# lyndonchan/wsss-analysis

Measured on AMD Instinct MI355X. Metric: images/sec CAM+CRF pseudo-labels, VOC2012 321x321, higher is better.
Workload: dtype f16x3; 1 GPU; resnet50 CAM + dense-CRF (M=21, 10 mean-field iters), 321x321, batch 32 images (=64 samples) per GPU, image-sharded; batch_images=32, num_classes=20, parallelism=image-sharded x1, no collective, steps_per_rank=239

## Files before the change

include/wsscam.h:

```cpp
#ifndef WSSCAM_H
#define WSSCAM_H

#include <stddef.h>
#include <stdint.h>

#ifdef __cplusplus
extern "C" {
#endif

#define WSC_VERSION 100

typedef enum wsc_status {
    WSC_OK = 0,
    WSC_ERR_INVALID = -1,
    WSC_ERR_NO_DEVICE = -2,
    WSC_ERR_HIP = -3,
    WSC_ERR_MISSING_KEY = -4,
    WSC_ERR_SHAPE = -5,
    WSC_ERR_NOMEM = -6,
    WSC_ERR_KEY_RANGE = -7,
    WSC_ERR_CAPACITY = -8,
    WSC_ERR_RANGE = -9
} wsc_status;

// ... 17 lines not shown
} wsc_precision;

typedef struct wsc_ctx wsc_ctx;
typedef struct wsc_net wsc_net;
typedef enum {
    WSC_OPT_CRF_GAUSS_ON_CHIP = 0,
    WSC_OPT_CRF_FUSED_BLUR = 1,
    WSC_OPT_CRF_BLUR_ON_CHIP = 2,
    WSC_OPT_CRF_RANK_BALLOT = 3,
    WSC_OPT_CRF_EMBED_FULL = 4,
    WSC_OPT_RW_TILED = 5,
    WSC_OPT_STEM_POOL_FUSED = 6,
    WSC_OPT_CONV_WINDOW = 7,
    WSC_OPT_CAM_HEAD_STREAM = 8,
    WSC_OPT_CRF_MSG_IN_UPDATE = 9,
    WSC_OPT_COUNT = 10
} wsc_option;

typedef struct wsc_crf wsc_crf;
typedef struct wsc_crf_v wsc_crf_v;

typedef struct wsc_tensor_desc {
    const char *name;
    const float *data;
    int32_t ndim;
    int64_t shape[4];
} wsc_tensor_desc;


int wsc_version(void);
const char *wsc_last_error(void);
// ... 384 lines not shown
```

profiles/conv_layer_table.py:

```python
import re
import sqlite3
import sys


def resnet50_layers(S):
    def o(h, k, s, p):
        return (h + 2 * p - k) // s + 1

    L = []
    h = o(S, 7, 2, 3)
    L.append(("stem 7x7 s2 3->64", h, 3, 64, 7))
    h = o(h, 3, 2, 1)
    inp = 64
    for li, (planes, blocks, stride) in enumerate(((64, 3, 1), (128, 4, 2), (256, 6, 2), (512, 3, 1)), 1):
        for b in range(blocks):
            s = stride if b == 0 else 1
            ho = o(h, 3, s, 1)
            n = "layer%d.%d." % (li, b)
            L.append((n + "conv1 1x1 %d->%d" % (inp, planes), h, inp, planes, 1))
            L.append((n + "conv2 3x3 %d s%d" % (planes, s), ho, planes, planes, 3))
            if b == 0:
                L.append((n + "conv3+proj 1x1 (%d+%d)->%d" % (planes, inp, planes * 4), ho, planes + inp, planes * 4, 1))
            else:
                L.append((n + "conv3 1x1 %d->%d +res" % (planes, planes * 4), ho, planes, planes * 4, 1))
# ... 17 lines not shown
def main(db, N=64, S=321, planes=1):
    c = sqlite3.connect(db)
    tabs = [r[0] for r in c.execute("select name from sqlite_master where type='table'")]
    kd = [t for t in tabs if "kernel_dispatch" in t][0]
    ks = [t for t in tabs if "kernel_symbol" in t][0]
    rows = c.execute("select s.kernel_name, d.start, d.end, d.grid_size_x / d.workgroup_size_x, d.group_segment_size "
                     "from %s d join %s s on d.kernel_id = s.id order by d.start" % (kd, ks)).fetchall()
    start = [i for i, r in enumerate(rows) if "nchw_to_nhwc4" in r[0]][-1]
    convs = [r for r in rows[start:] if "conv_igemm_kernel" in r[0] or "stem_pool_kernel" in r[0] or "cam_head_kernel" in r[0]]
    layers = resnet50_layers(S)
    if "stem_pool_kernel" in convs[0][0]:
        layers[0] = ("stem 7x7 s2 3->64 + maxpool (fused)",) + layers[0][1:]
    print("%-44s %8s %8s %9s %7s %6s" % ("layer", "us", "TFLOP/s", "act TB/s", "blocks", "LDS KB"))
    tot = 0.0
    pos = 0
    for (name, ho, cin, cout, k) in layers:
        M = N * ho * ho
        nd = n_dispatches(M, cin, cout, k, planes=planes)
        rs = convs[pos:pos + nd]
        pos += nd
        us = sum(r[2] - r[1] for r in rs) / 1000.0
        tot += us
        fl = 2.0 * M * cout * k * k * cin
        by = 2.0 * M * cout * (2 if "+res" in name else 1) + 2.0 * N * (ho * (2 if "s2" in name else 1)) ** 2 * cin
        if "fused" in name:
            by = 8.0 * N * S * S + 2.0 * N * ((ho + 1) // 2) ** 2 * cout
        by *= planes
        print("%-44s %8.1f %8.0f %9.2f %7s %6s" % (name, us, fl / us / 1e6, by / us / 1e6, "+".join(str(r[3]) for r in rs),
                                                    "/".join("%.0f" % (r[4] / 1024.0) for r in rs)))
    print("conv kernels total %.1f us" % tot)


if __name__ == "__main__":
    main(sys.argv[1], *(int(v) for v in sys.argv[2:]))
```

wsss-analysis_amd/csrc/common.h:

```cpp
#pragma once
#include <hip/hip_runtime.h>
#include <assert.h>
#include <stdint.h>
#include <map>
#include <string>
#include <unordered_map>
#include <vector>

#include "../../include/wsscam.h"

typedef uint16_t bf16_t;

typedef __bf16 bf16x8_t __attribute__((ext_vector_type(8)));
typedef _Float16 f16x8_t __attribute__((ext_vector_type(8)));
typedef float f32x16_t __attribute__((ext_vector_type(16)));
typedef float f32x4_t __attribute__((ext_vector_type(4)));

__host__ __device__ inline bf16_t f32_to_bf16(float f) {
    union { float f; uint32_t u; } v;
    v.f = f;
    uint32_t u = v.u;
    if ((u & 0x7fffffffu) > 0x7f800000u) return (bf16_t)((u >> 16) | 0x40);
    u += 0x7fffu + ((u >> 16) & 1u);
    return (bf16_t)(u >> 16);
// ... 106 lines not shown
    hipStream_t stream = nullptr;
    bool own_stream = false;
    int num_cus = 0;
    std::string arch;
    void *ws = nullptr;
    size_t ws_bytes = 0;
    static constexpr int PIN_SLOTS = 8;
    struct PinSlot {
        void *p = nullptr;
        size_t bytes = 0;
        hipEvent_t ev = nullptr;
        bool busy = false;
    };
    PinSlot pin_ring[PIN_SLOTS];
    int pin_next = 0;
    int opt[WSC_OPT_COUNT] = {1, 1, 1, 0, 0, -1, 1, 1, 1, 1};
    void *zero_page = nullptr;
    unsigned *range_host = nullptr, *range_dev = nullptr;
    hipEvent_t ev0 = nullptr, ev1 = nullptr;
    hipEvent_t join_ev = nullptr;
    hipEvent_t marks[8] = {};
    bool mark_set[8] = {};
    hipStream_t aux_stream = nullptr;
    hipEvent_t fork_ev = nullptr, aux_done_ev = nullptr;
    bool profiling = false;
    std::vector<WscProfRecord> prof;
    std::vector<hipEvent_t> prof_pool;
    std::multimap<size_t, void *> free_blocks;
    std::unordered_map<void *, size_t> live_blocks;
    WscGaussCache *gauss_cache = nullptr;
    int scratch_fill = -1;
// ... 182 lines not shown
    const float *s1, *b1;
    const float *s2, *b2;
    Act res;
    Act y;
    float *y_f32;
    int N, H, W, Cin, Ho, Wo, Cout, CoutPad;
    int kh, kw, stride, pad;
    int dil = 1;
    int relu;
    ConvForm form;
    wsc_precision prec;
    int generic;
    int ldy;
    Act x2;
    int H2, W2, C2, stride2;
    bool operands_match() const {
        for (const Act *a : {&x, &res, &y, &x2})
            if (*a && a->prec != prec) return false;
        return true;
    }
};
int conv_igemm_launch(wsc_ctx *ctx, const ConvLaunch &p);
int conv_f32_launch(wsc_ctx *ctx, const ConvLaunch &p);
int launch_cam_head(wsc_ctx *ctx, Act x, int M, int K, const bf16_t *w, int Kw, int CoutPad, const float *s1, const float *b1,
                    int C, int relu, float *y);

inline int wsc_grid_for(long long total, int block = 256, int cap = 256 * 16) {
    long long g = (total + block - 1) / block;
    if (g > cap) g = cap;
    if (g < 1) g = 1;
    return (int)g;
}
inline unsigned *layer_door(wsc_ctx *ctx, wsc_precision prec) { return conv_fmt(prec) == 1 ? ctx->range_dev : nullptr; }
int launch_nchw_to_nhwc4(wsc_ctx *ctx, const float *x, int N, int H, int W, Act y, unsigned *range);
void stem_pool_input_dims(int H, int W, int *Hp, int *Wp);
int launch_stem_pool(wsc_ctx *ctx, Act x, int N, int H, int W, const bf16_t *w, int Kw, const float *s1, const float *b1, int relu,
                     Act y);
// ... 141 lines not shown
```

wsss-analysis_amd/csrc/conv_igemm.hip:

```cpp
#include "common.h"

#include <type_traits>

namespace {

constexpr int BK = 64;

struct ConvKArgs {
    const bf16_t *x, *x_lo, *w;
    const float *s1, *b1, *s2, *b2;
    const bf16_t *res, *res_lo;
    bf16_t *y, *y_lo;
    float *y_f32;
    int H, W, Cin, Ho, Wo, Cout;
    int ldy;
    int kh, kw, stride, pad, relu;
    int M, HoWo;
    int m_base, m_end;
    unsigned div_howo_mul, div_howo_s1, div_howo_s2, div_wo_mul, div_wo_s1, div_wo_s2;
    int cchunks;
    int dil;
    int ksteps_base;
    int nk;
    int Kw;
    int Kbase;
    int ntiles_n, nblocks;
    const bf16_t *zero;
    int spare1;
    long long lo_delta;
    const bf16_t *x2;
    long long lo_delta2;
    int cc2, H2, W2, C2, stride2;
    int ldx;
    int win_npix;
    int spare2, spare3;
    unsigned *range;
};

__device__ __forceinline__ int lds_off(int row, int slot) {
    return row * 128 + ((slot ^ ((row >> 1) & 7)) << 4);
}

__device__ __forceinline__ void decode_row(const ConvKArgs &p, int m, int &n, int &ho, int &wo) {
    const unsigned t1 = __umulhi(p.div_howo_mul, (unsigned)m);
    n = (int)((t1 + (((unsigned)m - t1) >> p.div_howo_s1)) >> p.div_howo_s2);
    const int rem = m - n * p.HoWo;
    const unsigned t2 = __umulhi(p.div_wo_mul, (unsigned)rem);
    ho = (int)((t2 + (((unsigned)rem - t2) >> p.div_wo_s1)) >> p.div_wo_s2);
    wo = rem - ho * p.Wo;
}

template <int BM, int BN, int MODE, int SPLIT, int ET, int STAGES, int FAST = 0, int WPT = 0>
__global__ __launch_bounds__(BM * 2, (STAGES == 1 && FAST != 0) ? 4 : 2) void conv_igemm_kernel(ConvKArgs p) {
    constexpr bool GLDS = MODE == 0;
    constexpr int WMT = BM == 256 ? 128 : 64;
    constexpr bool FEPI = (FAST & 1) != 0, PW = (FAST & 2) != 0;
    constexpr bool WIN = WPT > 0;
    static_assert(!WIN || (SPLIT == 2 && BM == 128 && STAGES == 2 && FAST == 1), "LDS window: single-staged split, 128-row tile");
    static_assert(FAST == 0 || (SPLIT != 1 && ET == 1 && (MODE == 0 || FAST == 1)),
                  "FAST paths: f16, one plane or the single-staged split; the pointwise prologue belongs to the LDS-DMA layers");
    static_assert(SPLIT != 2 || (MODE == 0 && STAGES == 2), "single-staged split: LDS-DMA layers, two LDS buffers");
    static_assert(STAGES == 2 || SPLIT == 0, "one LDS buffer serves a one-K-step layer, which a layer of three K segments never is");
    constexpr int CK = SPLIT == 2 ? 32 : 64;
    constexpr int NT = BM * 2;
    constexpr int NW = BM / 32;
    constexpr int WR = BM / WMT;
    constexpr int WC = NW / WR;
    constexpr int WN = BN / WC;
// ... 516 lines not shown
        }
    } else {
        load_tile(0);
        store_lds(0);
        __syncthreads();
        for (int kt = 0; kt < nk; ++kt) {
            const int cur = kt & 1;
            const bool more = kt + 1 < nk;
            if (more) load_tile(kt + 1);
            compute(cur);
            if (more) store_lds(cur ^ 1);
            __syncthreads();
        }
    }

    constexpr int TPR = BN / 8;
    constexpr int RPP = NT / TPR;
    constexpr int NPASS = BM / RPP;
    const int c8 = t % TPR;
    const int r0 = t / TPR;
    const int c = n0 + c8 * 8;
    const bool cok = c < p.Cout;
    const bool full = c + 8 <= p.Cout;
    const bool has_res = p.res != nullptr && full;
    constexpr bool PRE_ALL = WMT == 64 && !(STAGES == 1 && FEPI);
    constexpr int NHALF_R = STAGES == 1 ? BM / 64 : (WMT == 128 ? BM / 128 : 1);
    constexpr int NRES = PRE_ALL ? NPASS : NPASS / NHALF_R;
    uint4 rres[NRES], rres_lo[NRES];
    auto fetch_res = [&](int first_pass) {
#pragma unroll
// ... 190 lines not shown
                    if (SPLIT) *reinterpret_cast<uint4 *>(p.y_lo + oy) = make_uint4(lw[0], lw[1], lw[2], lw[3]);
                }
            }
        }
    }
    if (ET && (ovf & 0x80008000u)) *p.range = (unsigned)p.Cout;
}

typedef void (*ConvKernel)(ConvKArgs);
struct ConvVariant {
    ConvKernel kernel;
    int bm, bn;
    int lds;
    int cls;
};
template <int BM, int BN, int MODE, int SPLIT, int ET, int STAGES, int FAST = 0, int WPT = 0>
ConvVariant variant() {
    constexpr int A_BYTES = BM * BK * 2, B_BYTES = BN * BK * 2;
    constexpr int PIPE = WPT > 0 ? WPT * 4096 + STAGES * B_BYTES : STAGES * (A_BYTES + B_BYTES);
    constexpr int EPI = (STAGES == 1 ? 64 : (BM == 256 ? 128 : BM)) * (BN + 4) * 4;
    constexpr int LDS = PIPE > EPI ? PIPE : EPI;
    static_assert(LDS <= 160 * 1024, "LDS budget of a CU");
    return {conv_igemm_kernel<BM, BN, MODE, SPLIT, ET, STAGES, FAST, WPT>, BM, BN, LDS,
            MODE != 0 ? WSC_K_CONV_SMALLCIN : (BM == 256 ? WSC_K_CONV256 : (BN == 128 ? WSC_K_CONV128 : WSC_K_CONV64))};
}
template <int BM, int BN, int MODE, int ET, int FAST = 0>
ConvVariant one_plane(bool one_kstep) {
    if constexpr (BM == 128)
        if (one_kstep) return variant<BM, BN, MODE, 0, ET, 1, FAST>();
    return variant<BM, BN, MODE, 0, ET, 2, FAST>();
}
template <int BM, int BN>
ConvVariant select_variant(ConvForm form, wsc_precision prec, int fast, bool one_kstep, int wpt) {
    if constexpr (BM == 128) {
        auto small = [&](auto mode) {
            constexpr int MODE = decltype(mode)::value;
            switch (prec) {
            case WSC_PREC_BF16: return one_plane<128, BN, MODE, 0>(one_kstep);
            case WSC_PREC_BF16X3: return variant<128, BN, MODE, 1, 0, 2>();
            case WSC_PREC_F16: return fast ? one_plane<128, BN, MODE, 1, 1>(one_kstep) : one_plane<128, BN, MODE, 1>(one_kstep);
            default: return variant<128, BN, MODE, 1, 1, 2>();
            }
        };
        if (form == CONV_FORM_SMALL2) return small(std::integral_constant<int, 1>{});
        if (form == CONV_FORM_SMALL4) return small(std::integral_constant<int, 2>{});
        if (wpt == 8) return variant<128, BN, 0, 2, 1, 2, 1, 8>();
        if (wpt == 10) return variant<128, BN, 0, 2, 1, 2, 1, 10>();
    }
    ConvVariant v;
    switch (prec) {
    case WSC_PREC_BF16: v = one_plane<BM, BN, 0, 0>(one_kstep); break;
    case WSC_PREC_BF16X3: v = variant<BM, BN, 0, 1, 0, 2>(); break;
    case WSC_PREC_F16:
        v = fast == 3 ? one_plane<BM, BN, 0, 1, 3>(one_kstep) : (fast ? one_plane<BM, BN, 0, 1, 1>(one_kstep) : one_plane<BM, BN, 0, 1>(one_kstep));
        break;
    default:
        v = fast == 3 ? variant<BM, BN, 0, 2, 1, 2, 3>() : (fast ? variant<BM, BN, 0, 2, 1, 2, 1>() : variant<BM, BN, 0, 2, 1, 2>());
        break;
    }
    if (form == CONV_FORM_STEM_ROWS) v.cls = WSC_K_CONV_SMALLCIN;
    return v;
}
ConvVariant conv_variant(int bm, int bn, ConvForm form, wsc_precision prec, int fast, bool one_kstep, int wpt = 0) {
    if (bm == 256) return select_variant<256, 256>(form, prec, fast, one_kstep, wpt);
    return bn == 128 ? select_variant<128, 128>(form, prec, fast, one_kstep, wpt) : select_variant<128, 64>(form, prec, fast, one_kstep, wpt);
}

}

int conv_igemm_launch(wsc_ctx *ctx, const ConvLaunch &p) {
    if (p.prec == WSC_PREC_F32) return conv_f32_launch(ctx, p);
    WSC_CHECK(p.operands_match(), WSC_ERR_INVALID, "conv: an operand is not of the layer's precision %d", (int)p.prec);
    const int split = conv_split(p.prec), fmt = conv_fmt(p.prec);
    const bool dma = conv_form_dma(p.form);
    if (p.form == CONV_FORM_STEM_ROWS)
        WSC_CHECK(split == 2 && p.Cin == 4 && p.pad == 0 && p.kw <= 7 && (p.stride & 1) == 0, WSC_ERR_INVALID,
                  "conv: the padded-stem form needs split 2, a 4-channel padded input, kw <= 7 and an even stride");
    else if (p.form == CONV_FORM_GENERIC) WSC_CHECK(p.Cin % 64 == 0, WSC_ERR_INVALID, "conv: Cin=%d not a multiple of 64", p.Cin);
    else WSC_CHECK(p.Cin == 4, WSC_ERR_INVALID, "conv: small-Cin mode needs a 4-channel activation");
    const ConvKLayout k = conv_k_layout(p.kh, p.kw, p.Cin, p.form, p.prec);
    const bool single_staged = k.interleaved;
    ConvKArgs a = {};
// ... 6 lines not shown
    a.win_npix = 0;
    a.ldx = p.Cin; a.x2 = nullptr; a.lo_delta2 = 0; a.cc2 = 0; a.H2 = a.W2 = a.C2 = 0; a.stride2 = 1;
    a.kh = p.kh; a.kw = k.kw_steps; a.stride = p.stride; a.pad = p.pad; a.relu = p.relu;
    a.M = p.N * p.Ho * p.Wo;
    a.HoWo = p.Ho * p.Wo;
    conv_fastdiv((unsigned)(a.HoWo > 0 ? a.HoWo : 1), &a.div_howo_mul, &a.div_howo_s1, &a.div_howo_s2);
    conv_fastdiv((unsigned)(p.Wo > 0 ? p.Wo : 1), &a.div_wo_mul, &a.div_wo_s1, &a.div_wo_s2);
    WSC_CHECK(p.dil >= 1, WSC_ERR_INVALID, "conv: dilation %d", p.dil);
    const int dil = (p.kh == 1 && p.kw == 1) ? 1 : p.dil;
    WSC_CHECK(dil == 1 || (p.form == CONV_FORM_GENERIC && !p.x2), WSC_ERR_INVALID,
              "conv: dilation %d needs a generic layer (Cin %% 64 == 0) with one input", dil);
    a.dil = dil;
    a.cchunks = k.cchunks; a.ksteps_base = k.ksteps_base;
    a.Kbase = k.Kbase; a.Kw = k.Kw; a.nk = k.nk;
    a.lo_delta = single_staged ? (long long)(a.x_lo - a.x) : 0;
    if (p.x2) {
        const int K1 = p.Cin - p.C2;
        WSC_CHECK(split != 1 && dma && p.kh == 1 && p.kw == 1 && p.stride == 1 && p.pad == 0 && K1 > 0 &&
                  K1 % 64 == 0 && p.C2 % 64 == 0 && p.stride2 >= 1 && (p.Ho - 1) * p.stride2 < p.H2 && (p.Wo - 1) * p.stride2 < p.W2 &&
                  (!single_staged || p.x2.h16_lo() != nullptr),
                  WSC_ERR_INVALID, "conv: a second input needs a 1x1 / stride 1 layer, channel counts in multiples of 64 and no bf16x3");
        a.x2 = p.x2.h16();
        a.lo_delta2 = single_staged ? (long long)(p.x2.h16_lo() - a.x2) : 0;
        a.cc2 = K1 / k.ck;
        a.H2 = p.H2; a.W2 = p.W2; a.C2 = p.C2; a.stride2 = p.stride2;
        a.ldx = K1;
    }
    WSC_CHECK(p.CoutPad % 64 == 0, WSC_ERR_INVALID, "conv: CoutPad=%d not a multiple of 64", p.CoutPad);
    const int BN = conv_tile_bn(p.CoutPad);
    a.zero = (const bf16_t *)ctx->zero_page;
    a.range = ctx->range_dev;
    int fast = 0;
    if (!p.generic && dil == 1 && fmt && (split == 0 || single_staged) && p.y && p.y_f32 == nullptr &&
        p.Cout == p.CoutPad && (long long)a.M * a.ldy < (1ll << 31)) {
        fast = 1;
        if (dma && p.kh == 1 && p.kw == 1 && p.pad == 0 && p.stride == 1) fast = 3;
    }
    if (a.M == 0) return WSC_OK;
    auto launch = [&](const ConvVariant &v, int m_base, int m_end) -> int {
        ConvKArgs b = a;
        b.m_base = m_base;
        b.m_end = m_end;
        b.ntiles_n = p.CoutPad / v.bn;
        b.nblocks = ((m_end - m_base + v.bm - 1) / v.bm) * b.ntiles_n;
        WSC_TRY(wsc_set_max_dynamic_lds(ctx, reinterpret_cast<const void *>(v.kernel), v.lds));
        const double flops = 2.0 * (m_end - m_base) * a.Cout * (p.form == CONV_FORM_GENERIC ? (double)p.kh * p.kw * p.Cin : (double)p.kh * p.kw * 3);
        WscKernelTimer timer(ctx, v.cls, flops);
        hipLaunchKernelGGL(v.kernel, dim3(b.nblocks), dim3(v.bm * 2), v.lds, ctx->stream, b);
        WSC_HIP(hipGetLastError());
        return WSC_OK;
    };
    const bool one_kstep = a.nk == 1;
    const long long blocks_sq = ((a.M + 255) / 256) * (long long)(p.CoutPad / 256);
    bool square = dma && p.CoutPad % 256 == 0 && a.nk >= 4 && blocks_sq >= 192;
    if (split == 2 && !fast) square = false;
    if (split == 2 && a.nk < 16) square = false;
    if (square) {
        const ConvVariant sq = conv_variant(256, 256, p.form, p.prec, fast, one_kstep);
        const long long rounds = blocks_sq / ctx->num_cus, rem = blocks_sq - rounds * ctx->num_cus;
        if (rounds >= 1 && rem > 0 && rem * 2 <= ctx->num_cus && ctx->num_cus > 0) {
            const int big_rows = (int)((rounds * ctx->num_cus) / (p.CoutPad / 256));
            WSC_TRY(launch(sq, 0, big_rows * 256));
            return launch(conv_variant(128, BN, p.form, p.prec, fast, one_kstep), big_rows * 256, a.M);
        }
        return launch(sq, 0, a.M);
    }
    int wpt = 0;
    if (single_staged && fast == 1 && dil == 1 && p.kh == 3 && p.kw == 3 && p.stride == 1 && p.pad == 1 && !p.x2 &&
        p.Ho == p.H && p.Wo == p.W && ctx->opt[WSC_OPT_CONV_WINDOW] != 0) {
        const long long need = 127 + 2ll * p.W + 3 + 1;
        const long long npix = (long long)p.N * p.H * p.W;
        if (need <= 320 && npix < (1ll << 30) && a.lo_delta >= 0 && npix * p.Cin + a.lo_delta < (1ll << 33) && (a.lo_delta & 7) == 0) {
            a.win_npix = (int)npix;
            wpt = need <= 256 ? 8 : 10;
        }
    }
    return launch(conv_variant(128, BN, p.form, p.prec, fast, one_kstep, wpt), 0, a.M);
}
```

wsss-analysis_amd/csrc/net.hip:

```cpp
#include "common.h"

#include <algorithm>
#include <cmath>
#include <cstring>
#include <unordered_map>

namespace {

struct HostTensor {
    const float *data;
    int ndim;
    int64_t shape[4];
    int64_t numel() const {
        int64_t n = 1;
        for (int i = 0; i < ndim; ++i) n *= shape[i];
        return n;
    }
};
typedef std::unordered_map<std::string, HostTensor> Dict;

struct ConvW {
    void *w = nullptr;
    float *s1 = nullptr, *b1 = nullptr, *s2 = nullptr, *b2 = nullptr;
    int Cin = 0, Cout = 0, CoutPad = 0, kh = 1, kw = 1, stride = 1, pad = 0, relu = 0;
// ... 723 lines not shown
}

bool stem_pool_fused(const wsc_ctx *ctx, const wsc_net *net) {
    if (net->ops.empty() || net->ops[0].type != OP_CONV || net->ops[0].in >= 0 || net->convs[net->ops[0].conv].form != CONV_FORM_STEM_ROWS)
        return false;
    const ConvW &c0 = net->convs[net->ops[0].conv];
    bool tapped = false;
    for (int tp : net->taps) tapped = tapped || tp == 0;
    return ctx->opt[WSC_OPT_STEM_POOL_FUSED] && net->ops.size() > 1 && net->ops[1].type == OP_POOL &&
           net->ops[1].in == net->ops[0].out && net->ops[1].rule == POOL_TORCH && !net->ops[1].avg && net->ops[1].pk == 3 &&
           net->ops[1].ps == 2 && net->ops[1].pp == 1 &&
           c0.kh == 7 && c0.kw == 7 && c0.stride == 2 && c0.pad == 3 && c0.Cout == 64 && c0.s2 == nullptr &&
           net->ops[0].res < 0 && conv_fmt(net->prec) == 1 && !tapped;
}

struct TraceSink {
    const long long *off;
    float *out;
};

int run_backbone(wsc_ctx *ctx, const wsc_net *net, const float *x_dev, int N, int S, size_t extra_bytes, Act *feat, int *hf, int *wf,
                 void **extra, std::vector<Act> *taps = nullptr, int SW = 0, bool nhwc_in = false, Act *spare = nullptr,
                 const TraceSink *trace = nullptr, Act *xin_out = nullptr) {
    if (SW <= 0) SW = S;
    Plan pl;
    WSC_TRY(plan_dims(net, N, S, SW, &pl));
    int in_h = S, in_w = SW, in_pad = 0;
    bool fused_stem = false;
    if (!net->ops.empty() && net->ops[0].type == OP_CONV && net->ops[0].in < 0 && net->convs[net->ops[0].conv].form == CONV_FORM_STEM_ROWS) {
        const ConvW &c0 = net->convs[net->ops[0].conv];
// ... 9 lines not shown
    void *ws;
    WSC_TRY(wsc_ctx_workspace(ctx, act_bytes(in_elems, net->prec) + 4 * act_bytes(pl.max_act, net->prec) + align_up(extra_bytes, 256), &ws));
    char *p = (char *)ws;
    const Act xin = act_carve(p, in_elems, net->prec);
    Act buf[4];
    for (Act &b : buf) b = act_carve(p, pl.max_act, net->prec);
    if (taps)
        for (int op : net->taps) taps->push_back(act_carve(p, pl.out_elems(N, op), net->prec));
    *extra = (void *)p;

    if (nhwc_in) {
        WSC_CHECK(in_pad == 0, WSC_ERR_INVALID, "internal: an NHWC input has no padded-stem form");
        WSC_TRY(launch_nhwc3_to_nhwc4(ctx, x_dev, N, S, SW, xin));
    } else if (in_pad > 0) WSC_TRY(launch_nchw_to_nhwc4_pad(ctx, x_dev, N, S, SW, in_h, in_w, in_pad, xin, ctx->range_dev));
    else WSC_TRY(launch_nchw_to_nhwc4(ctx, x_dev, N, S, SW, xin, ctx->range_dev));
    for (size_t i = 0; i < net->ops.size(); ++i) {
        const Op &op = net->ops[i];
        const OpDims &d = pl.ops[i];
        const Act src = op.in < 0 ? xin : buf[op.in];
        if (fused_stem && i == 0) continue;
        if (fused_stem && i == 1) {
            const ConvW &c0 = net->convs[net->ops[0].conv];
            WSC_TRY(launch_stem_pool(ctx, xin, N, S, SW, (const bf16_t *)c0.w, conv_k_layout(c0.kh, c0.kw, c0.Cin, c0.form, net->prec).Kw, c0.s1,
                                     c0.b1, c0.relu, buf[op.out]));
        } else if (op.type == OP_CONV) {
            const ConvW &c = net->convs[op.conv];
            ConvLaunch L = conv_launch(c, net->prec);
            L.x = src;
            if (op.res >= 0) L.res = buf[op.res];
            L.y = buf[op.out].at(op.coff);
            L.ldy = op.pitch;
            if (op.in2 >= 0) {
                L.x2 = buf[op.in2];
                L.H2 = d.H2; L.W2 = d.W2; L.C2 = d.C2; L.stride2 = op.ps;
            }
            L.N = N; L.H = d.H; L.W = d.W; L.Ho = d.Ho; L.Wo = d.Wo;
            if (c.form == CONV_FORM_STEM_ROWS && op.in < 0) on_padded_input(L, in_h, in_w);
            WSC_TRY(conv_igemm_launch(ctx, L));
        } else if (op.type == OP_GATHER) {
            WSC_TRY(launch_gather_strided(ctx, src, N, d.H, d.W, d.C, op.ps, d.Ho, d.Wo, buf[op.out].at(op.coff), op.pitch));
        } else {
            PoolGeom g;
            WSC_CHECK(pool_geom(op.rule, op.pk, op.ps, op.pp, op.avg, d.H, d.W, &g), WSC_ERR_INVALID, "internal: a pool plan_dims let through");
            WSC_TRY(launch_pool(ctx, src, N, d.H, d.W, d.C, g, buf[op.out]));
        }
        if (trace && trace->off[i] >= 0) WSC_TRY(launch_act_to_f32(ctx, buf[op.out], pl.out_elems(N, (int)i), trace->out + trace->off[i]));
        if (taps)
            for (size_t k = 0; k < net->taps.size(); ++k)
                if (net->taps[k] == (int)i) {
                    const size_t nb = pl.out_elems(N, (int)i) * conv_elem_bytes(net->prec);
                    WSC_HIP(hipMemcpyAsync((*taps)[k].hi, buf[op.out].hi, nb, hipMemcpyDeviceToDevice, ctx->stream));
                    if (buf[op.out].lo) WSC_HIP(hipMemcpyAsync((*taps)[k].lo, buf[op.out].lo, nb, hipMemcpyDeviceToDevice, ctx->stream));
                }
    }
    *feat = buf[net->final_buf];
    if (xin_out) *xin_out = xin;
    if (spare) *spare = buf[net->final_buf == 3 ? 2 : 3];
    *hf = pl.hf;
    *wf = pl.wf;
    return WSC_OK;
}

int run_classifier(wsc_ctx *ctx, const wsc_net *net, Act feat, Act spare, int N, int count, int sample_stride, int hf, int wf,
                   float *score_dev) {
    int hw = hf * wf;
    if (net->cls_max && net->cls_pool_set) {
        const PoolSpec &ps = net->cls_pool;
        PoolGeom g;
// ... 176 lines not shown
        const OpDims &d = pl->ops[i];
        wsc_trace_op t = {};
        set_label(t, op.label);
        t.in = producer(op.in);
        t.in2 = t.res = WSC_TRACE_NONE;
        t.Ho = d.Ho; t.Wo = d.Wo; t.pitch = d.Co; t.coff = op.coff; t.C = d.Co;
        if (op.type == OP_CONV) {
            const ConvW &c = net->convs[op.conv];
            t.kind = WSC_TRACE_CONV;
            t.C = c.Cout;
            if (op.in2 >= 0) t.in2 = producer(op.in2);
            if (op.res >= 0) t.res = producer(op.res);
            t.kh = c.kh; t.kw = c.kw; t.stride = c.stride; t.pad = c.pad; t.dil = c.dil; t.relu = c.relu;
            t.affine2 = c.s2 != nullptr;
            t.stride2 = op.in2 >= 0 ? op.ps : 0;
            t.fused_next = fused && i == 0;
        } else if (op.type == OP_GATHER) {
            t.kind = WSC_TRACE_GATHER;
            t.C = d.C;
            t.stride = op.ps;
        } else {
            t.kind = WSC_TRACE_POOL;
            t.pool_rule = (int)op.rule; t.pool_k = op.pk; t.pool_stride = op.ps; t.pool_pad = op.pp; t.pool_avg = op.avg;
        }
        writer[op.out] = (int)i;
        out->push_back(t);
    }
    if (net->head.w != nullptr) {
        wsc_trace_op t = {};
        set_label(t, "head");
        t.kind = WSC_TRACE_HEAD;
// ... 1210 lines not shown
```

wsss-analysis_amd/wsscam/_lib.py:

```python
import ctypes
import os
import re
import threading

import numpy as np

_HERE = os.path.dirname(os.path.abspath(__file__))
LIB_PATH = os.path.join(_HERE, "libwsscam.so")
HEADER_PATH = os.path.normpath(os.path.join(_HERE, "..", "..", "include", "wsscam.h"))

WSC_OK = 0
WSC_ERR_INVALID = -1
WSC_ERR_NO_DEVICE = -2
WSC_ERR_HIP = -3
WSC_ERR_MISSING_KEY = -4
WSC_ERR_SHAPE = -5
WSC_ERR_NOMEM = -6
WSC_ERR_KEY_RANGE = -7
WSC_ERR_CAPACITY = -8
WSC_ERR_RANGE = -9

ARCH_RESNET50_CAM = 0
ARCH_VGG16_CAM = 1
ARCH_M7_CAM = 2
ARCH_RESNET50_IRN = 3
ARCH_VGG16_IRN = 4
ARCH_M7_IRN = 5
ARCH_DEEPLAB_LFOV = 6
ARCH_DEEPLAB_ASPP = 7

PREC_BF16 = 0
PREC_BF16X3 = 1
PREC_F16 = 2
PREC_F16X3 = 3
PREC_F32 = 4
OPT_CRF_GAUSS_ON_CHIP, OPT_CRF_FUSED_BLUR, OPT_CRF_BLUR_ON_CHIP, OPT_CRF_RANK_BALLOT, OPT_CRF_EMBED_FULL, OPT_RW_TILED, \
    OPT_STEM_POOL_FUSED, OPT_CONV_WINDOW, OPT_CAM_HEAD_STREAM, OPT_CRF_MSG_IN_UPDATE = range(10)
OPT_DEFAULTS = {OPT_CRF_GAUSS_ON_CHIP: 1, OPT_CRF_FUSED_BLUR: 1, OPT_CRF_BLUR_ON_CHIP: 1, OPT_CRF_RANK_BALLOT: 0,
                OPT_CRF_EMBED_FULL: 0, OPT_RW_TILED: -1, OPT_STEM_POOL_FUSED: 1, OPT_CONV_WINDOW: 1, OPT_CAM_HEAD_STREAM: 1,
                OPT_CRF_MSG_IN_UPDATE: 1}
CONV_GENERIC = 0x100


class WscError(RuntimeError):
    def __init__(self, status, message):
        super().__init__("libwsscam error %d: %s" % (status, message))
        self.status = status


class TensorDesc(ctypes.Structure):
    _fields_ = [
        ("name", ctypes.c_char_p),
        ("data", ctypes.POINTER(ctypes.c_float)),
        ("ndim", ctypes.c_int32),
        ("shape", ctypes.c_int64 * 4),
# ... 1421 lines not shown
```

Baseline: 2646 images/s.

## Fuse bottleneck 3x3 conv2 with following 1x1 conv3 and residual into one kernel

Adds a fused variant of the windowed implicit-GEMM conv kernel. It keeps the 3x3 conv2 output tile (all 64 channels, f16x3 hi/lo) in LDS and runs the 1x1 conv3 expansion to 256 channels, with BN, residual add and ReLU, in the kernel tail. This targets the layer1 bottlenecks, where Cout is 64, and drops the conv2 activation write/read and one launch per block. In exchange the kernel uses more LDS and registers, has extra barriers in the tail, and is limited to two blocks per CU. The default of -1 turns it on only for untraced runs.

Measured after the change: 2663 images/s, median of 6. About the same (+0.7%).

```diff
diff --git a/include/wsscam.h b/include/wsscam.h
--- a/include/wsscam.h
+++ b/include/wsscam.h
@@ -55,7 +55,8 @@
     WSC_OPT_CONV_WINDOW = 7,
     WSC_OPT_CAM_HEAD_STREAM = 8,
     WSC_OPT_CRF_MSG_IN_UPDATE = 9,
-    WSC_OPT_COUNT = 10
+    WSC_OPT_CONV_FUSE23 = 10,
+    WSC_OPT_COUNT = 11
 } wsc_option;
 
 typedef struct wsc_crf wsc_crf;
diff --git a/profiles/conv_layer_table.py b/profiles/conv_layer_table.py
--- a/profiles/conv_layer_table.py
+++ b/profiles/conv_layer_table.py
@@ -55,7 +55,11 @@
     print("%-44s %8s %8s %9s %7s %6s" % ("layer", "us", "TFLOP/s", "act TB/s", "blocks", "LDS KB"))
     tot = 0.0
     pos = 0
-    for (name, ho, cin, cout, k) in layers:
+    skip = False
+    for li, (name, ho, cin, cout, k) in enumerate(layers):
+        if skip:
+            skip = False
+            continue
         M = N * ho * ho
         nd = n_dispatches(M, cin, cout, k, planes=planes)
         rs = convs[pos:pos + nd]
@@ -64,6 +68,12 @@
         tot += us
         fl = 2.0 * M * cout * k * k * cin
         by = 2.0 * M * cout * (2 if "+res" in name else 1) + 2.0 * N * (ho * (2 if "s2" in name else 1)) ** 2 * cin
+        if k == 3 and re.search(r"conv_igemm_kernel(<(\d+,\s*){8}1>|I(Li\d+E){8}Li1EE)", rs[0][0]):
+            n3, _, cin3, cout3, _ = layers[li + 1]
+            name = name.split("conv2")[0] + "conv2+conv3 one kernel %d->%d +res" % (cin, cout3)
+            fl += 2.0 * M * cout3 * cin3
+            by = 2.0 * M * cin + 2.0 * M * cout3 * 2
+            skip = True
         if "fused" in name:
             by = 8.0 * N * S * S + 2.0 * N * ((ho + 1) // 2) ** 2 * cout
         by *= planes
diff --git a/wsss-analysis_amd/csrc/common.h b/wsss-analysis_amd/csrc/common.h
--- a/wsss-analysis_amd/csrc/common.h
+++ b/wsss-analysis_amd/csrc/common.h
@@ -144,7 +144,7 @@
     };
     PinSlot pin_ring[PIN_SLOTS];
     int pin_next = 0;
-    int opt[WSC_OPT_COUNT] = {1, 1, 1, 0, 0, -1, 1, 1, 1, 1};
+    int opt[WSC_OPT_COUNT] = {1, 1, 1, 0, 0, -1, 1, 1, 1, 1, -1};
     void *zero_page = nullptr;
     unsigned *range_host = nullptr, *range_dev = nullptr;
     hipEvent_t ev0 = nullptr, ev1 = nullptr;
@@ -357,6 +357,9 @@
     int ldy;
     Act x2;
     int H2, W2, C2, stride2;
+    const void *w3;
+    const float *s3, *b3;
+    int Cout3;
     bool operands_match() const {
         for (const Act *a : {&x, &res, &y, &x2})
             if (*a && a->prec != prec) return false;
@@ -364,6 +367,7 @@
     }
 };
 int conv_igemm_launch(wsc_ctx *ctx, const ConvLaunch &p);
+bool conv_fuse23_fits(const wsc_ctx *ctx, const ConvLaunch &c2, const ConvLaunch &c3, long long lo_delta);
 int conv_f32_launch(wsc_ctx *ctx, const ConvLaunch &p);
 int launch_cam_head(wsc_ctx *ctx, Act x, int M, int K, const bf16_t *w, int Kw, int CoutPad, const float *s1, const float *b1,
                     int C, int relu, float *y);
diff --git a/wsss-analysis_amd/csrc/conv_igemm.hip b/wsss-analysis_amd/csrc/conv_igemm.hip
--- a/wsss-analysis_amd/csrc/conv_igemm.hip
+++ b/wsss-analysis_amd/csrc/conv_igemm.hip
@@ -35,6 +35,9 @@
     int win_npix;
     int spare2, spare3;
     unsigned *range;
+    const bf16_t *w3;
+    const float *s3, *b3;
+    int Cout3, Kw3;
 };
 
 __device__ __forceinline__ int lds_off(int row, int slot) {
@@ -50,8 +53,9 @@
     wo = rem - ho * p.Wo;
 }
 
-template <int BM, int BN, int MODE, int SPLIT, int ET, int STAGES, int FAST = 0, int WPT = 0>
+template <int BM, int BN, int MODE, int SPLIT, int ET, int STAGES, int FAST = 0, int WPT = 0, int FUSE = 0>
 __global__ __launch_bounds__(BM * 2, (STAGES == 1 && FAST != 0) ? 4 : 2) void conv_igemm_kernel(ConvKArgs p) {
+    static_assert(!FUSE || (WPT > 0 && BN == 64), "fused 1 x 1 layer: behind a window variant whose tile holds every output channel");
     constexpr bool GLDS = MODE == 0;
     constexpr int WMT = BM == 256 ? 128 : 64;
     constexpr bool FEPI = (FAST & 1) != 0, PW = (FAST & 2) != 0;
@@ -598,6 +602,188 @@
         }
     }
 
+    if constexpr (FUSE) {
+        constexpr int NK2 = BN / 32;
+        constexpr int A2_BYTES = BM * 128;
+        constexpr int BC = 64;
+        constexpr int NCH = 4 * BN / BC;
+        constexpr int B2_BYTES = BC * 128;
+        constexpr int B2_OFF = NK2 * A2_BYTES, CT2_OFF = B2_OFF + NK2 * B2_BYTES;
+        constexpr int CT2 = BC + 4;
+        constexpr int NWP = NK2 * BC * 8 / NT;
+        constexpr int TPR2 = BC / 8, RPP2 = NT / TPR2, PPG = 64 / RPP2, NPS = BM / RPP2;
+        static_assert(MI == 2 && NI == 1 && WC == 2 && BC == WC * 32 && PPG * RPP2 == 64 && (NK2 * BC * 8) % NT == 0, "fused tail layout");
+        auto lds_barrier = [] { asm volatile("s_waitcnt lgkmcnt(0)\n\ts_barrier" ::: "memory"); };
+        const int c8 = t % TPR2, r0 = t / TPR2;
+        u32x4_t wq[NWP];
+        auto w3_load = [&](int ch) {
+#pragma unroll
+            for (int i = 0; i < NWP; ++i) {
+                const int g = i * NT + t;
+                const int kt = g / (BC * 8), rr = (g % (BC * 8)) >> 3, ss = g & 7;
+                wq[i] = *reinterpret_cast<const u32x4_t *>(p.w3 + ((long long)(ch * BC + rr) * p.Kw3 + kt * 64 + ss * 8));
+            }
+        };
+        auto w3_store = [&]() {
+#pragma unroll
+            for (int i = 0; i < NWP; ++i) {
+                const int g = i * NT + t;
+                const int kt = g / (BC * 8), rr = (g % (BC * 8)) >> 3, ss = g & 7;
+                *reinterpret_cast<u32x4_t *>(smem + B2_OFF + kt * B2_BYTES + lds_off(rr, ss)) = wq[i];
+            }
+        };
+        uint4 rn[NPS], rnl[NPS];
+        auto res_load = [&](int ch, int g) {
+            const unsigned c = (unsigned)(ch * BC + c8 * 8);
+#pragma unroll
+            for (int i = g * PPG; i < (g + 1) * PPG; ++i) {
+                const int m = m0 + i * RPP2 + r0;
+                const int mc = m < p.m_end ? m : p.m_end - 1;
+                rn[i] = *reinterpret_cast<const uint4 *>(p.res + ((unsigned)mc * (unsigned)p.Cout3 + c));
+                rnl[i] = *reinterpret_cast<const uint4 *>(p.res_lo + ((unsigned)mc * (unsigned)p.Cout3 + c));
+            }
+        };
+        f32x4_t sbn[4];
+        auto sb_load = [&](int ch) {
+            const int c = ch * BC + c8 * 8;
+            sbn[0] = *reinterpret_cast<const f32x4_t *>(p.s3 + c);
+            sbn[1] = *reinterpret_cast<const f32x4_t *>(p.s3 + c + 4);
+            sbn[2] = *reinterpret_cast<const f32x4_t *>(p.b3 + c);
+            sbn[3] = *reinterpret_cast<const f32x4_t *>(p.b3 + c + 4);
+        };
+        w3_load(0);
+        unsigned ovf2 = 0u;
+        {
+            const float sat2 = p.relu ? 0.f : -65504.f;
+            const int col = wn * WN + l31;
+            const float sc = p.s1[col], sf = p.b1[col];
+            char *dst = smem + (col >> 5) * A2_BYTES + (col & 7) * 2;
+            const int cs = (col & 31) >> 3;
+#pragma unroll
+            for (int mi = 0; mi < MI; ++mi)
+#pragma unroll
+                for (int r = 0; r < 16; ++r) {
+                    const int row = wm * WMT + mi * 32 + (r & 3) + 8 * (r >> 2) + 4 * kgrp;
+                    const float v = acc[mi][0][r] * sc + sf;
+                    const float c0 = __builtin_amdgcn_fmed3f(v, sat2, 65504.f);
+                    const _Float16 h0 = (_Float16)c0;
+                    const _Float16 l0 = (_Float16)(c0 - (float)h0);
+                    const uint16_t hbits = __builtin_bit_cast(uint16_t, h0);
+                    if (m0 + row < p.m_end) ovf2 |= half2_at_ceiling((unsigned)hbits);
+                    *reinterpret_cast<uint16_t *>(dst + lds_off(row, cs)) = hbits;
+                    *reinterpret_cast<uint16_t *>(dst + lds_off(row, 4 + cs)) = __builtin_bit_cast(uint16_t, l0);
+                }
+        }
+        w3_store();
+        if (NCH > 1) w3_load(1);
+        sb_load(0);
+        res_load(0, 0);
+        res_load(0, 1);
+        lds_barrier();
+        float *ct2 = reinterpret_cast<float *>(smem + CT2_OFF);
+        unsigned ovf3 = 0u;
+#pragma unroll
+        for (int ch = 0; ch < NCH; ++ch) {
+            f32x16_t a2[MI];
+#pragma unroll
+            for (int mi = 0; mi < MI; ++mi)
+#pragma unroll
+                for (int r = 0; r < 16; ++r) a2[mi][r] = 0.f;
+#pragma unroll
+            for (int kt = 0; kt < NK2; ++kt)
+#pragma unroll
+                for (int sl = 0; sl < 2; ++sl) {
+                    u32x4_t ah[MI], al[MI];
+#pragma unroll
+                    for (int mi = 0; mi < MI; ++mi) {
+                        const int row = wm * WMT + mi * 32 + l31;
+                        ah[mi] = *reinterpret_cast<const u32x4_t *>(smem + kt * A2_BYTES + lds_off(row, sl * 2 + kgrp));
+                        al[mi] = *reinterpret_cast<const u32x4_t *>(smem + kt * A2_BYTES + lds_off(row, 4 + sl * 2 + kgrp));
+                    }
+                    const u32x4_t bh = *reinterpret_cast<const u32x4_t *>(smem + B2_OFF + kt * B2_BYTES + lds_off(wn * 32 + l31, sl * 2 + kgrp));
+                    const u32x4_t bl = *reinterpret_cast<const u32x4_t *>(smem + B2_OFF + kt * B2_BYTES + lds_off(wn * 32 + l31, 4 + sl * 2 + kgrp));
+#pragma unroll
+                    for (int mi = 0; mi < MI; ++mi) mfma(al[mi], bh, a2[mi]);
+#pragma unroll
+                    for (int mi = 0; mi < MI; ++mi) mfma(ah[mi], bl, a2[mi]);
+#pragma unroll
+                    for (int mi = 0; mi < MI; ++mi) mfma(ah[mi], bh, a2[mi]);
+                }
+            const int c = ch * BC + c8 * 8;
+            float s3[8], b3[8];
+#pragma unroll
+            for (int j = 0; j < 4; ++j) {
+                s3[j] = sbn[0][j];
+                s3[4 + j] = sbn[1][j];
+                b3[j] = sbn[2][j];
+                b3[4 + j] = sbn[3][j];
+            }
+#pragma unroll
+            for (int g = 0; g < 2; ++g) {
+                if (g > 0) lds_barrier();
+                if (wm == g) {
+#pragma unroll
+                    for (int mi = 0; mi < MI; ++mi)
+#pragma unroll
+                        for (int r = 0; r < 16; ++r)
+                            ct2[(mi * 32 + (r & 3) + 8 * (r >> 2) + 4 * kgrp) * CT2 + wn * 32 + l31] = a2[mi][r];
+                }
+                lds_barrier();
+                if (g == 0) {
+                    if (ch + 1 < NCH) w3_store();
+                    if (ch + 2 < NCH) w3_load(ch + 2);
+                    if (ch + 1 < NCH) sb_load(ch + 1);
+                }
+#pragma unroll
+                for (int pp = 0; pp < PPG; ++pp) {
+                    const int ri = g * PPG + pp;
+                    const int lrow_e = pp * RPP2 + r0;
+                    const int m = m0 + g * 64 + lrow_e;
+                    float v[8];
+                    const f32x4_t q0 = *reinterpret_cast<const f32x4_t *>(ct2 + lrow_e * CT2 + c8 * 8);
+                    const f32x4_t q1 = *reinterpret_cast<const f32x4_t *>(ct2 + lrow_e * CT2 + c8 * 8 + 4);
+#pragma unroll
+                    for (int j = 0; j < 4; ++j) {
+                        v[j] = q0[j] * s3[j] + b3[j];
+                        v[4 + j] = q1[j] * s3[4 + j] + b3[4 + j];
+                    }
+                    const uint32_t rw[4] = {rn[ri].x, rn[ri].y, rn[ri].z, rn[ri].w};
+#pragma unroll
+                    for (int j = 0; j < 4; ++j) {
+                        v[2 * j] += f16_to_f32((bf16_t)(rw[j] & 0xffffu));
+                        v[2 * j + 1] += f16_to_f32((bf16_t)(rw[j] >> 16));
+                    }
+                    const uint32_t rl[4] = {rnl[ri].x, rnl[ri].y, rnl[ri].z, rnl[ri].w};
+#pragma unroll
+                    for (int j = 0; j < 4; ++j) {
+                        v[2 * j] += f16_to_f32((bf16_t)(rl[j] & 0xffffu));
+                        v[2 * j + 1] += f16_to_f32((bf16_t)(rl[j] >> 16));
+                    }
+                    uint32_t hw[4], lw[4];
+#pragma unroll
+                    for (int j = 0; j < 4; ++j) {
+                        const float c0 = __builtin_amdgcn_fmed3f(v[2 * j], 0.f, 65504.f), c1 = __builtin_amdgcn_fmed3f(v[2 * j + 1], 0.f, 65504.f);
+                        const _Float16 h0 = (_Float16)c0;
+                        const _Float16 h1 = (_Float16)c1;
+                        hw[j] = (uint32_t)__builtin_bit_cast(uint16_t, h0) | ((uint32_t)__builtin_bit_cast(uint16_t, h1) << 16);
+                        const _Float16 l0 = (_Float16)(c0 - (float)h0), l1 = (_Float16)(c1 - (float)h1);
+                        lw[j] = (uint32_t)__builtin_bit_cast(uint16_t, l0) | ((uint32_t)__builtin_bit_cast(uint16_t, l1) << 16);
+                    }
+                    if (m < p.m_end) {
+                        ovf3 |= half2_at_ceiling(hw[0]) | half2_at_ceiling(hw[1]) | half2_at_ceiling(hw[2]) | half2_at_ceiling(hw[3]);
+                        *reinterpret_cast<uint4 *>(p.y + ((unsigned)m * (unsigned)p.ldy + (unsigned)c)) = make_uint4(hw[0], hw[1], hw[2], hw[3]);
+                        *reinterpret_cast<uint4 *>(p.y_lo + ((unsigned)m * (unsigned)p.ldy + (unsigned)c)) = make_uint4(lw[0], lw[1], lw[2], lw[3]);
+                    }
+                }
+                if (ch + 1 < NCH) res_load(ch + 1, g);
+            }
+            lds_barrier();
+        }
+        if (ovf2 & 0x8000u) *p.range = (unsigned)p.Cout;
+        if (ovf3 & 0x80008000u) *p.range = (unsigned)p.Cout3;
+        return;
+    }
+
     constexpr int TPR = BN / 8;
     constexpr int RPP = NT / TPR;
     constexpr int NPASS = BM / RPP;
@@ -818,14 +1004,15 @@
     int lds;
     int cls;
 };
-template <int BM, int BN, int MODE, int SPLIT, int ET, int STAGES, int FAST = 0, int WPT = 0>
+template <int BM, int BN, int MODE, int SPLIT, int ET, int STAGES, int FAST = 0, int WPT = 0, int FUSE = 0>
 ConvVariant variant() {
     constexpr int A_BYTES = BM * BK * 2, B_BYTES = BN * BK * 2;
     constexpr int PIPE = WPT > 0 ? WPT * 4096 + STAGES * B_BYTES : STAGES * (A_BYTES + B_BYTES);
     constexpr int EPI = (STAGES == 1 ? 64 : (BM == 256 ? 128 : BM)) * (BN + 4) * 4;
-    constexpr int LDS = PIPE > EPI ? PIPE : EPI;
-    static_assert(LDS <= 160 * 1024, "LDS budget of a CU");
-    return {conv_igemm_kernel<BM, BN, MODE, SPLIT, ET, STAGES, FAST, WPT>, BM, BN, LDS,
+    constexpr int TAIL = FUSE ? (BN / 32) * (BM * 128 + 64 * 128) + 64 * (64 + 4) * 4 : 0;
+    constexpr int LDS = TAIL ? (PIPE > TAIL ? PIPE : TAIL) : (PIPE > EPI ? PIPE : EPI);
+    static_assert(LDS <= 160 * 1024 && (!FUSE || LDS <= 80 * 1024), "LDS budget of a CU (fused: two blocks)");
+    return {conv_igemm_kernel<BM, BN, MODE, SPLIT, ET, STAGES, FAST, WPT, FUSE>, BM, BN, LDS,
             MODE != 0 ? WSC_K_CONV_SMALLCIN : (BM == 256 ? WSC_K_CONV256 : (BN == 128 ? WSC_K_CONV128 : WSC_K_CONV64))};
 }
 template <int BM, int BN, int MODE, int ET, int FAST = 0>
@@ -835,7 +1022,7 @@
     return variant<BM, BN, MODE, 0, ET, 2, FAST>();
 }
 template <int BM, int BN>
-ConvVariant select_variant(ConvForm form, wsc_precision prec, int fast, bool one_kstep, int wpt) {
+ConvVariant select_variant(ConvForm form, wsc_precision prec, int fast, bool one_kstep, int wpt, bool fuse) {
     if constexpr (BM == 128) {
         auto small = [&](auto mode) {
             constexpr int MODE = decltype(mode)::value;
@@ -848,6 +1035,10 @@
         };
         if (form == CONV_FORM_SMALL2) return small(std::integral_constant<int, 1>{});
         if (form == CONV_FORM_SMALL4) return small(std::integral_constant<int, 2>{});
+        if constexpr (BN == 64) {
+            if (fuse && wpt == 8) return variant<128, 64, 0, 2, 1, 2, 1, 8, 1>();
+            if (fuse && wpt == 10) return variant<128, 64, 0, 2, 1, 2, 1, 10, 1>();
+        }
         if (wpt == 8) return variant<128, BN, 0, 2, 1, 2, 1, 8>();
         if (wpt == 10) return variant<128, BN, 0, 2, 1, 2, 1, 10>();
     }
@@ -865,11 +1056,32 @@
     if (form == CONV_FORM_STEM_ROWS) v.cls = WSC_K_CONV_SMALLCIN;
     return v;
 }
-ConvVariant conv_variant(int bm, int bn, ConvForm form, wsc_precision prec, int fast, bool one_kstep, int wpt = 0) {
-    if (bm == 256) return select_variant<256, 256>(form, prec, fast, one_kstep, wpt);
-    return bn == 128 ? select_variant<128, 128>(form, prec, fast, one_kstep, wpt) : select_variant<128, 64>(form, prec, fast, one_kstep, wpt);
+ConvVariant conv_variant(int bm, int bn, ConvForm form, wsc_precision prec, int fast, bool one_kstep, int wpt = 0, bool fuse = false) {
+    if (bm == 256) return select_variant<256, 256>(form, prec, fast, one_kstep, wpt, false);
+    return bn == 128 ? select_variant<128, 128>(form, prec, fast, one_kstep, wpt, false) : select_variant<128, 64>(form, prec, fast, one_kstep, wpt, fuse);
 }
 
+int conv_window_groups(const ConvLaunch &p, long long lo_delta) {
+    const long long need = 127 + 2ll * p.W + 3 + 1;
+    const long long npix = (long long)p.N * p.H * p.W;
+    if (need <= 320 && npix < (1ll << 30) && lo_delta >= 0 && npix * p.Cin + lo_delta < (1ll << 33) && (lo_delta & 7) == 0) return need <= 256 ? 8 : 10;
+    return 0;
+}
+bool fuse23_first_fits(const wsc_ctx *ctx, const ConvLaunch &p, int Cout3, long long lo_delta) {
+    const long long M = (long long)p.N * p.Ho * p.Wo;
+    return p.prec == WSC_PREC_F16X3 && p.form == CONV_FORM_GENERIC && !p.generic && p.kh == 3 && p.kw == 3 && p.stride == 1 && p.pad == 1 &&
+           p.dil == 1 && p.Ho == p.H && p.Wo == p.W && p.Cin % 64 == 0 && p.Cout == 64 && p.CoutPad == 64 && p.s2 == nullptr &&
+           p.y_f32 == nullptr && !p.x2 && Cout3 == 4 * p.Cout && M > 0 && M * Cout3 < (1ll << 31) &&
+           ctx->opt[WSC_OPT_CONV_WINDOW] != 0 && conv_window_groups(p, lo_delta) != 0;
+}
+
+}
+
+bool conv_fuse23_fits(const wsc_ctx *ctx, const ConvLaunch &c2, const ConvLaunch &c3, long long lo_delta) {
+    const bool second = c3.prec == c2.prec && c3.form == CONV_FORM_GENERIC && !c3.generic && c3.kh == 1 && c3.kw == 1 && c3.stride == 1 &&
+                        c3.pad == 0 && c3.Cin == c2.Cout && c3.Cout == c3.CoutPad && c3.relu == 1 && c3.s2 == nullptr && c3.y_f32 == nullptr &&
+                        !c3.x2 && c3.N == c2.N && c3.H == c2.Ho && c3.W == c2.Wo && c3.Ho == c3.H && c3.Wo == c3.W;
+    return second && fuse23_first_fits(ctx, c2, c3.Cout, lo_delta);
 }
 
 int conv_igemm_launch(wsc_ctx *ctx, const ConvLaunch &p) {
@@ -906,6 +1118,16 @@
     a.cchunks = k.cchunks; a.ksteps_base = k.ksteps_base;
     a.Kbase = k.Kbase; a.Kw = k.Kw; a.nk = k.nk;
     a.lo_delta = single_staged ? (long long)(a.x_lo - a.x) : 0;
+    const bool fuse = p.w3 != nullptr;
+    if (fuse) {
+        WSC_CHECK(fuse23_first_fits(ctx, p, p.Cout3, a.lo_delta) && p.s3 && p.b3 && p.res && p.y && p.y.h16_lo() && p.res.h16_lo() &&
+                  (p.ldy == 0 || p.ldy == p.Cout3), WSC_ERR_INVALID, "conv: no fused 3x3 -> 1x1 kernel for this pair of layers (conv_fuse23_fits)");
+        a.w3 = (const bf16_t *)p.w3; a.s3 = p.s3; a.b3 = p.b3; a.Cout3 = p.Cout3;
+        a.Kw3 = conv_k_layout(1, 1, p.Cout, CONV_FORM_GENERIC, p.prec).Kw;
+        a.ldy = p.Cout3;
+    } else {
+        WSC_CHECK(!p.s3 && !p.b3 && !p.Cout3, WSC_ERR_INVALID, "conv: a fused 1x1 layer without its weights");
+    }
     if (p.x2) {
         const int K1 = p.Cin - p.C2;
         WSC_CHECK(split != 1 && dma && p.kh == 1 && p.kw == 1 && p.stride == 1 && p.pad == 0 && K1 > 0 &&
@@ -936,7 +1158,8 @@
         b.ntiles_n = p.CoutPad / v.bn;
         b.nblocks = ((m_end - m_base + v.bm - 1) / v.bm) * b.ntiles_n;
         WSC_TRY(wsc_set_max_dynamic_lds(ctx, reinterpret_cast<const void *>(v.kernel), v.lds));
-        const double flops = 2.0 * (m_end - m_base) * a.Cout * (p.form == CONV_FORM_GENERIC ? (double)p.kh * p.kw * p.Cin : (double)p.kh * p.kw * 3);
+        const double flops = 2.0 * (m_end - m_base) * a.Cout * (p.form == CONV_FORM_GENERIC ? (double)p.kh * p.kw * p.Cin : (double)p.kh * p.kw * 3) +
+                             (fuse ? 2.0 * (m_end - m_base) * (double)p.Cout3 * p.Cout : 0.0);
         WscKernelTimer timer(ctx, v.cls, flops);
         hipLaunchKernelGGL(v.kernel, dim3(b.nblocks), dim3(v.bm * 2), v.lds, ctx->stream, b);
         WSC_HIP(hipGetLastError());
@@ -960,12 +1183,9 @@
     int wpt = 0;
     if (single_staged && fast == 1 && dil == 1 && p.kh == 3 && p.kw == 3 && p.stride == 1 && p.pad == 1 && !p.x2 &&
         p.Ho == p.H && p.Wo == p.W && ctx->opt[WSC_OPT_CONV_WINDOW] != 0) {
-        const long long need = 127 + 2ll * p.W + 3 + 1;
-        const long long npix = (long long)p.N * p.H * p.W;
-        if (need <= 320 && npix < (1ll << 30) && a.lo_delta >= 0 && npix * p.Cin + a.lo_delta < (1ll << 33) && (a.lo_delta & 7) == 0) {
-            a.win_npix = (int)npix;
-            wpt = need <= 256 ? 8 : 10;
-        }
-    }
-    return launch(conv_variant(128, BN, p.form, p.prec, fast, one_kstep, wpt), 0, a.M);
+        wpt = conv_window_groups(p, a.lo_delta);
+        if (wpt) a.win_npix = (int)((long long)p.N * p.H * p.W);
+    }
+    WSC_CHECK(!fuse || (wpt != 0 && BN == 64 && fast == 1), WSC_ERR_INVALID, "conv: the fused 3x3 -> 1x1 pair did not get its window variant");
+    return launch(conv_variant(128, BN, p.form, p.prec, fast, one_kstep, wpt, fuse), 0, a.M);
 }
diff --git a/wsss-analysis_amd/csrc/net.hip b/wsss-analysis_amd/csrc/net.hip
--- a/wsss-analysis_amd/csrc/net.hip
+++ b/wsss-analysis_amd/csrc/net.hip
@@ -761,6 +761,26 @@
            net->ops[0].res < 0 && conv_fmt(net->prec) == 1 && !tapped;
 }
 
+ConvLaunch op_launch(const wsc_net *net, const Plan &pl, int N, size_t i) {
+    const OpDims &d = pl.ops[i];
+    ConvLaunch L = conv_launch(net->convs[net->ops[i].conv], net->prec);
+    L.N = N; L.H = d.H; L.W = d.W; L.Ho = d.Ho; L.Wo = d.Wo;
+    return L;
+}
+bool conv23_fused(const wsc_ctx *ctx, const wsc_net *net, const Plan &pl, int N, size_t i, bool per_op) {
+    const int sel = ctx->opt[WSC_OPT_CONV_FUSE23];
+    if (sel == 0 || (sel < 0 && per_op) || i + 1 >= net->ops.size()) return false;
+    const Op &o2 = net->ops[i], &o3 = net->ops[i + 1];
+    if (o2.type != OP_CONV || o3.type != OP_CONV) return false;
+    for (int tp : net->taps)
+        if (tp == (int)i) return false;
+    if (o2.in < 0 || o2.res >= 0 || o2.in2 >= 0 || o2.pitch != 0 || o3.in != o2.out || o3.in2 >= 0 || o3.pitch != 0 || o3.res < 0 ||
+        o3.res == o2.out || o3.res == o2.in || o3.out == o3.res || o3.out == o2.out)
+        return false;
+    const long long lo_delta = (long long)(act_bytes(pl.max_act, net->prec) / 2 / conv_elem_bytes(net->prec));
+    return conv_fuse23_fits(ctx, op_launch(net, pl, N, i), op_launch(net, pl, N, i + 1), lo_delta);
+}
+
 struct TraceSink {
     const long long *off;
     float *out;
@@ -800,11 +820,37 @@
         WSC_TRY(launch_nhwc3_to_nhwc4(ctx, x_dev, N, S, SW, xin));
     } else if (in_pad > 0) WSC_TRY(launch_nchw_to_nhwc4_pad(ctx, x_dev, N, S, SW, in_h, in_w, in_pad, xin, ctx->range_dev));
     else WSC_TRY(launch_nchw_to_nhwc4(ctx, x_dev, N, S, SW, xin, ctx->range_dev));
+    auto observe = [&](size_t i) -> int {
+        const Op &op = net->ops[i];
+        if (trace && trace->off[i] >= 0) WSC_TRY(launch_act_to_f32(ctx, buf[op.out], pl.out_elems(N, (int)i), trace->out + trace->off[i]));
+        if (taps)
+            for (size_t k = 0; k < net->taps.size(); ++k)
+                if (net->taps[k] == (int)i) {
+                    const size_t nb = pl.out_elems(N, (int)i) * conv_elem_bytes(net->prec);
+                    WSC_HIP(hipMemcpyAsync((*taps)[k].hi, buf[op.out].hi, nb, hipMemcpyDeviceToDevice, ctx->stream));
+                    if (buf[op.out].lo) WSC_HIP(hipMemcpyAsync((*taps)[k].lo, buf[op.out].lo, nb, hipMemcpyDeviceToDevice, ctx->stream));
+                }
+        return WSC_OK;
+    };
     for (size_t i = 0; i < net->ops.size(); ++i) {
         const Op &op = net->ops[i];
         const OpDims &d = pl.ops[i];
         const Act src = op.in < 0 ? xin : buf[op.in];
         if (fused_stem && i == 0) continue;
+        if (conv23_fused(ctx, net, pl, N, i, trace != nullptr)) {
+            const Op &o3 = net->ops[i + 1];
+            const ConvW &c3 = net->convs[o3.conv];
+            ConvLaunch L = op_launch(net, pl, N, i);
+            L.x = src;
+            L.w3 = c3.w; L.s3 = c3.s1; L.b3 = c3.b1; L.Cout3 = c3.Cout;
+            L.res = buf[o3.res];
+            L.y = buf[op.out];
+            WSC_TRY(conv_igemm_launch(ctx, L));
+            std::swap(buf[op.out], buf[o3.out]);
+            WSC_TRY(observe(i + 1));
+            ++i;
+            continue;
+        }
         if (fused_stem && i == 1) {
             const ConvW &c0 = net->convs[net->ops[0].conv];
             WSC_TRY(launch_stem_pool(ctx, xin, N, S, SW, (const bf16_t *)c0.w, conv_k_layout(c0.kh, c0.kw, c0.Cin, c0.form, net->prec).Kw, c0.s1,
@@ -830,14 +876,7 @@
             WSC_CHECK(pool_geom(op.rule, op.pk, op.ps, op.pp, op.avg, d.H, d.W, &g), WSC_ERR_INVALID, "internal: a pool plan_dims let through");
             WSC_TRY(launch_pool(ctx, src, N, d.H, d.W, d.C, g, buf[op.out]));
         }
-        if (trace && trace->off[i] >= 0) WSC_TRY(launch_act_to_f32(ctx, buf[op.out], pl.out_elems(N, (int)i), trace->out + trace->off[i]));
-        if (taps)
-            for (size_t k = 0; k < net->taps.size(); ++k)
-                if (net->taps[k] == (int)i) {
-                    const size_t nb = pl.out_elems(N, (int)i) * conv_elem_bytes(net->prec);
-                    WSC_HIP(hipMemcpyAsync((*taps)[k].hi, buf[op.out].hi, nb, hipMemcpyDeviceToDevice, ctx->stream));
-                    if (buf[op.out].lo) WSC_HIP(hipMemcpyAsync((*taps)[k].lo, buf[op.out].lo, nb, hipMemcpyDeviceToDevice, ctx->stream));
-                }
+        WSC_TRY(observe(i));
     }
     *feat = buf[net->final_buf];
     if (xin_out) *xin_out = xin;
@@ -1044,7 +1083,7 @@
             t.kh = c.kh; t.kw = c.kw; t.stride = c.stride; t.pad = c.pad; t.dil = c.dil; t.relu = c.relu;
             t.affine2 = c.s2 != nullptr;
             t.stride2 = op.in2 >= 0 ? op.ps : 0;
-            t.fused_next = fused && i == 0;
+            t.fused_next = (fused && i == 0) || conv23_fused(ctx, net, *pl, N, i, true);
         } else if (op.type == OP_GATHER) {
             t.kind = WSC_TRACE_GATHER;
             t.C = d.C;
diff --git a/wsss-analysis_amd/wsscam/_lib.py b/wsss-analysis_amd/wsscam/_lib.py
--- a/wsss-analysis_amd/wsscam/_lib.py
+++ b/wsss-analysis_amd/wsscam/_lib.py
@@ -35,10 +35,10 @@
 PREC_F16X3 = 3
 PREC_F32 = 4
 OPT_CRF_GAUSS_ON_CHIP, OPT_CRF_FUSED_BLUR, OPT_CRF_BLUR_ON_CHIP, OPT_CRF_RANK_BALLOT, OPT_CRF_EMBED_FULL, OPT_RW_TILED, \
-    OPT_STEM_POOL_FUSED, OPT_CONV_WINDOW, OPT_CAM_HEAD_STREAM, OPT_CRF_MSG_IN_UPDATE = range(10)
+    OPT_STEM_POOL_FUSED, OPT_CONV_WINDOW, OPT_CAM_HEAD_STREAM, OPT_CRF_MSG_IN_UPDATE, OPT_CONV_FUSE23 = range(11)
 OPT_DEFAULTS = {OPT_CRF_GAUSS_ON_CHIP: 1, OPT_CRF_FUSED_BLUR: 1, OPT_CRF_BLUR_ON_CHIP: 1, OPT_CRF_RANK_BALLOT: 0,
                 OPT_CRF_EMBED_FULL: 0, OPT_RW_TILED: -1, OPT_STEM_POOL_FUSED: 1, OPT_CONV_WINDOW: 1, OPT_CAM_HEAD_STREAM: 1,
-                OPT_CRF_MSG_IN_UPDATE: 1}
+                OPT_CRF_MSG_IN_UPDATE: 1, OPT_CONV_FUSE23: -1}
 CONV_GENERIC = 0x100
 
 
```
